# succinctlabs/tendermintx

Hardware: AMD Instinct MI355X
Metric: skip-circuit witness-gen ms at VALIDATOR_SET_SIZE_MAX=128 (lower is better)
Workload: dtype int64; 1 GPU; SkipCircuit VALIDATOR_SET_SIZE_MAX=128, batch of 256 proofs over 1 GPU(s) (BASELINE configs[3] batch per GPU, weak-scaled), 100 validators in 128 lanes, 4 distinct validator set(s) per batch, 90% sign; n_max=128, proofs_total=256, proofs_per_gpu=256, workload_name=survey8d, parallelism=proof-sharded x1, no data-path collective

## Files before the change

### include/tmx.h

```cpp
#ifndef TMX_H
#define TMX_H
#include <stddef.h>
#include <stdint.h>

#ifdef __cplusplus
extern "C" {
#endif

#define TMX_KIND_SKIP 0
#define TMX_KIND_STEP 1

#define TMX_N_MAX_LIMIT 512

#define TMX_VALIDATOR_MESSAGE_BYTES_LENGTH_MAX 124
#define TMX_VALIDATOR_BYTE_LENGTH_MAX 46
#define TMX_PROTOBUF_CHAIN_ID_SIZE_BYTES 52
#define TMX_HEADER_PROOF_DEPTH 4

#define TMX_FLAG_SIGNED 1u
#define TMX_FLAG_PRESENT 2u

typedef enum {
  TMX_OK = 0,
  TMX_ERR_BAD_ARG = -1,
// ... 443 lines not shown
#define TMX_TRACE_SHA256_HELPER 128u
#define TMX_TRACE_SHA256_QUOTIENT 256u
int32_t tmx_air_sha256_helper_device(tmx_ctx* ctx, uint32_t log_rows, uint32_t n_proofs, const uint64_t* d_table, uint64_t* d_helper,
                                     void* hip_stream);
int32_t tmx_air_sha256_quotient_device(tmx_ctx* ctx, uint32_t log_n, uint32_t log_blowup, uint32_t cap_height, uint32_t n_proofs,
                                       const uint64_t* d_cols, const uint64_t* d_helper_cols, const uint64_t* d_cap, const uint64_t* d_cap_helper,
                                       uint64_t* d_quot, void* hip_stream);
int32_t tmx_air_sha256_verify_device(tmx_ctx* ctx, const tmx_batch_params* p, uint32_t k_trace, const uint64_t* d_caps, const uint64_t* d_proof,
                                     uint32_t* d_ok, void* hip_stream);
int32_t tmx_trace_commit_set_air_sha256_device(tmx_ctx* ctx, uint32_t section, uint64_t* d_cap_h, uint64_t* d_cap_q, void* hip_stream);

int32_t tmx_selftest_fe_invert(tmx_ctx* ctx, uint32_t n, const uint32_t* in_words, uint32_t* out_words);

int32_t tmx_selftest_f16(tmx_ctx* ctx, uint32_t n, uint32_t doublings, const uint32_t* in_words, uint32_t* out_words);

#ifdef __cplusplus
}
#endif
#endif
```

### tendermintx_amd/_lib.py

```python
import ctypes as C
import ctypes.util
import importlib.util
import os
import sys

_HERE = os.path.dirname(os.path.abspath(__file__))
LIB_PATH = os.environ.get("TMX_LIB") or os.path.join(_HERE, "libtmx.so")

KIND_SKIP, KIND_STEP = 0, 1
FLAG_SIGNED, FLAG_PRESENT = 1, 2
N_KERNELS = 4
KERNEL_NAMES = ("k_eddsa", "k_proof", "k_verdict", "k_serialize")
ED_STRIDE = 448
SEC_HINT, SEC_DERIVED, SEC_ALL = 1, 2, 3
PROOF_PATH_NONE, PROOF_PATH_TINY, PROOF_PATH_ROLES, PROOF_PATH_R168, PROOF_PATH_K256, PROOF_PATH_WIDE = range(6)
TRACE_LADDERS, TRACE_SHA512, TRACE_SHA256, TRACE_MATCH, TRACE_TREE, TRACE_HEADER, TRACE_ALL = 1, 2, 4, 8, 16, 32, 63
TRACE_LADDERS_QUOTIENT = 64
AIR_SHA256_HELPER_COLS, AIR_SHA256_CONSTRAINTS = 300, 315
TRACE_SHA256_HELPER, TRACE_SHA256_QUOTIENT = 128, 256


class ValidatorRec(C.Structure):
    _fields_ = [("pubkey", C.c_uint8 * 32), ("signature", C.c_uint8 * 64), ("message", C.c_uint8 * 124),
                ("message_byte_length", C.c_uint16), ("validator_byte_length", C.c_uint8), ("flags", C.c_uint8),
# ... 270 lines not shown
        L.tmx_batch_verify_device.argtypes = [C.c_void_p, C.POINTER(BatchParams), C.c_void_p, C.c_void_p, C.c_void_p, C.c_void_p]
        L.tmx_trace_commit_set_device.argtypes = [C.c_void_p, C.c_int32, C.c_uint32, C.c_uint32, C.c_uint32, C.c_uint32, C.c_void_p, C.c_void_p,
                                                  C.c_void_p]
        L.tmx_trace_commit_set_shape.argtypes = [C.c_void_p, C.POINTER(BatchParams), C.POINTER(C.c_uint32)]
        L.tmx_trace_commit_set_prove_device.argtypes = [C.c_void_p, C.POINTER(BatchParams), C.c_void_p, C.c_void_p]
        L.tmx_trace_commit_set_bytes.argtypes = [C.c_int32] + [C.c_uint32] * 7
        L.tmx_trace_commit_set_bytes.restype = C.c_uint64
        L.tmx_trace_commit_set_streamed_device.argtypes = [C.c_void_p, C.c_int32, C.c_uint32, C.c_uint32, C.c_uint32, C.c_uint32, C.c_uint32,
                                                           C.c_uint32, C.c_void_p, C.c_void_p, C.c_void_p]
        L.tmx_air_ladder_quotient_device.argtypes = [C.c_void_p, C.c_uint32, C.c_uint32, C.c_uint32, C.c_uint32, C.c_void_p, C.c_void_p, C.c_void_p,
                                                     C.c_void_p]
        L.tmx_air_ladder_quotient_range_device.argtypes = [C.c_void_p] + [C.c_uint32] * 7 + [C.c_void_p] * 4
        L.tmx_air_last_gamma.argtypes = [C.c_void_p, C.POINTER(C.c_uint64)]
        L.tmx_air_verify_device.argtypes = [C.c_void_p, C.POINTER(BatchParams), C.c_uint32, C.c_void_p, C.c_void_p, C.c_void_p, C.c_void_p]
        L.tmx_trace_commit_set_air_device.argtypes = [C.c_void_p, C.c_void_p, C.c_void_p]
    except AttributeError:
        if not os.environ.get("TMX_LIB"):
            raise
    L.tmx_selftest_fe_invert.argtypes = [C.c_void_p, C.c_uint32, C.c_void_p, C.c_void_p]
    L.tmx_selftest_f16.argtypes = [C.c_void_p, C.c_uint32, C.c_uint32, C.c_void_p, C.c_void_p]
    L.tmx_eddsa_lanes_device.argtypes = [C.c_void_p, C.c_uint32, C.c_void_p, C.c_void_p, C.c_void_p]
    L.tmx_finish_batch_device.argtypes = [C.c_void_p, C.c_int32, C.c_uint32, C.c_void_p, C.c_void_p, C.c_void_p, C.c_void_p,
                                          C.c_void_p, C.c_void_p, C.c_void_p]
    L.tmx_trace_commit_shape.argtypes = [C.c_int32, C.c_uint32, C.c_uint32, C.POINTER(C.c_uint32), C.POINTER(C.c_uint32)]
    L.tmx_trace_commit_device.argtypes = [C.c_void_p, C.c_int32, C.c_uint32, C.c_uint32, C.c_uint32, C.c_uint32, C.c_void_p, C.c_void_p, C.c_void_p]
    L.tmx_trace_commit_last_ms.argtypes = [C.c_void_p, C.POINTER(C.c_float)]
    L.tmx_shard_range.restype = None
    L.tmx_shard_range.argtypes = [C.c_uint64, C.c_uint32, C.c_uint32, C.POINTER(C.c_uint64), C.POINTER(C.c_uint64)]
    L.tmx_comm_unique_id.argtypes = [C.c_char_p]
    L.tmx_comm_create.argtypes = [C.c_void_p, C.c_char_p, C.c_uint32, C.c_uint32]
# ... 83 lines not shown
```

### tendermintx_amd/context.py

```python
import ctypes as C

import numpy as np

from . import _lib
from ._lib import KIND_SKIP, KIND_STEP, Config, Report, check


def _indices(indices):
    if isinstance(indices, np.ndarray):
        return np.ascontiguousarray(indices.reshape(-1), dtype=np.uint64)
    return np.array([int(i) for i in indices], dtype=np.uint64)


class Context:

    def __init__(self, n_max, chain_id=b"celestia", skip_max=100800, device=0, max_batch=1):
        self._L = _lib.lib()
        self.n_max, self.chain_id, self.skip_max, self.max_batch = int(n_max), bytes(chain_id), int(skip_max), int(max_batch)
        cfg = Config()
        cfg.n_max = self.n_max
        cfg.chain_id_len = len(self.chain_id)
        for i, b in enumerate(self.chain_id[:52]):
            cfg.chain_id[i] = b
        cfg.skip_max = self.skip_max
# ... 151 lines not shown
        for i, v in enumerate(values):
            for k in range(8):
                inp[i, k] = (int(v) >> (32 * k)) & 0xFFFFFFFF
        out = np.zeros((n, 16), dtype=np.uint32)
        check(self._L.tmx_selftest_fe_invert(self._h, n, inp.ctypes.data, out.ctypes.data), self._h)
        conv = lambda w: sum(int(w[k]) << (32 * k) for k in range(8))
        return [(conv(out[i, :8]), conv(out[i, 8:])) for i in range(n)]

    def selftest_f16(self, words, doublings):
        inp = np.ascontiguousarray(words, dtype=np.uint32)
        n = inp.shape[0]
        out = np.zeros((n, 256), dtype=np.uint32)
        check(self._L.tmx_selftest_f16(self._h, n, doublings, inp.ctypes.data, out.ctypes.data), self._h)
        return out

    def ntt_set_domain(self, root_2_32, coset_shift):
        check(self._L.tmx_ntt_set_domain(self._h, C.c_uint64(root_2_32), C.c_uint64(coset_shift)), self._h)

    def ntt_device(self, log_n, n_cols, d_in, d_out, inverse=False, stream=None):
        check(self._L.tmx_ntt_goldilocks_device(self._h, log_n, n_cols, d_in, d_out, 1 if inverse else 0, self._stream(stream)), self._h)

    def lde_device(self, log_n, log_blowup, n_cols, d_in, d_out, stream=None):
        check(self._L.tmx_lde_goldilocks_device(self._h, log_n, log_blowup, n_cols, d_in, d_out, self._stream(stream)), self._h)

    def poseidon_set_constants(self, round_constants=None, mds_circ=None, mds_diag=None):
        arr = lambda v, n: (C.c_uint64 * n)(*[int(x) for x in v]) if v is not None else None
        check(self._L.tmx_poseidon_set_constants(self._h, arr(round_constants, 360), arr(mds_circ, 12), arr(mds_diag, 12)), self._h)

    def poseidon_permute(self, states):
        a = np.ascontiguousarray(states, dtype=np.uint64).reshape(-1, 12)
# ... 355 lines not shown
```

### tendermintx_amd/csrc/api.cpp

```cpp
#include <hip/hip_runtime_api.h>

#include <algorithm>
#include <chrono>
#include <cstdio>
#include <cstdlib>
#include <cstring>
#include <mutex>
#include <string>
#include <thread>
#include <vector>

#include "kernels.h"
#include "air.h"
#include "fri.h"
#include "ntt.h"
#include "poseidon.h"
#include "trace.h"
#include "tmx.h"
#include "value.h"

using namespace tmx;

static thread_local std::string g_tls_err;

// ... 2065 lines not shown
  HIPCK(c, hipSetDevice(c->cfg.device));
  void *d_in = nullptr, *d_out = nullptr;
  hipError_t e = hipMalloc(&d_in, (size_t)n * 512);
  if (e == hipSuccess) e = hipMalloc(&d_out, (size_t)n * 1024);
  if (e == hipSuccess) e = hipMemcpy(d_in, in_words, (size_t)n * 512, hipMemcpyHostToDevice);
  if (e == hipSuccess) e = hipMemsetAsync(d_out, 0, (size_t)n * 1024, c->side2);
  if (e == hipSuccess) e = (hipError_t)launch_selftest_f16(n, doublings, d_in, d_out, c->side2);
  if (e == hipSuccess) e = hipStreamSynchronize(c->side2);
  if (e == hipSuccess) e = hipMemcpy(out_words, d_out, (size_t)n * 1024, hipMemcpyDeviceToHost);
  if (d_in) (void)hipFree(d_in);
  if (d_out) (void)hipFree(d_out);
  if (e != hipSuccess) return fail(c, TMX_ERR_HIP, std::string("tmx_selftest_f16: ") + hipGetErrorString(e));
  return TMX_OK;
}

int32_t tmx_selftest_fe_invert(tmx_ctx* c, uint32_t n, const uint32_t* in_words, uint32_t* out_words) {
  if (!c || !in_words || !out_words) return TMX_ERR_BAD_ARG;
  if (n == 0) return TMX_OK;
  HIPCK(c, hipSetDevice(c->cfg.device));
  void *d_in = nullptr, *d_out = nullptr;
  hipError_t e = hipMalloc(&d_in, (size_t)n * 32);
  if (e == hipSuccess) e = hipMalloc(&d_out, (size_t)n * 64);
  if (e == hipSuccess) e = hipMemcpy(d_in, in_words, (size_t)n * 32, hipMemcpyHostToDevice);
  if (e == hipSuccess) e = (hipError_t)launch_selftest_invert(n, d_in, d_out, c->side2);
  if (e == hipSuccess) e = hipStreamSynchronize(c->side2);
  if (e == hipSuccess) e = hipMemcpy(out_words, d_out, (size_t)n * 64, hipMemcpyDeviceToHost);
  if (d_in) (void)hipFree(d_in);
  if (d_out) (void)hipFree(d_out);
  if (e != hipSuccess) return fail(c, TMX_ERR_HIP, std::string("tmx_selftest_fe_invert: ") + hipGetErrorString(e));
  return TMX_OK;
// ... 2305 lines not shown
```

### tendermintx_amd/csrc/fe25519.hpp

```cpp
#pragma once
#include <hip/hip_runtime.h>
#include <stdint.h>

namespace tmx {

struct fe {
  int32_t v[10];
};

#define TMX_DEV __device__ __forceinline__
#ifdef TMX_FE_NOINLINE
#define TMX_FE_FN __device__ __noinline__
#else
#define TMX_FE_FN __device__ __forceinline__
#endif

TMX_DEV fe fe_zero() {
  fe r;
#pragma unroll
  for (int i = 0; i < 10; i++) r.v[i] = 0;
  return r;
}
TMX_DEV fe fe_one() {
  fe r = fe_zero();
// ... 119 lines not shown
  r.v[1] += c;
  return r;
}

TMX_DEV fe fe_from_words(const uint32_t w[8]) {
  fe r;
  const int start[10] = {0, 26, 51, 77, 102, 128, 153, 179, 204, 230};
#pragma unroll
  for (int i = 0; i < 10; i++) {
    const int s = start[i], bits = (i & 1) ? 25 : 26;
    const int wi = s >> 5, sh = s & 31;
    uint64_t two = (uint64_t)w[wi] | ((wi + 1 < 8) ? ((uint64_t)w[wi + 1] << 32) : 0);
    uint32_t val = (uint32_t)(two >> sh) & ((1u << bits) - 1);
    if (i == 9) val &= (1u << 25) - 1;
    r.v[i] = (int32_t)val;
  }
  return r;
}

TMX_DEV void fe_to_words(const fe& a, uint32_t w[8]) {
  int32_t h[10];
#pragma unroll
  for (int i = 0; i < 10; i++) h[i] = a.v[i];
#pragma unroll
  for (int i = 0; i < 10; i++) {
    const int bits = (i & 1) ? 25 : 26;
    int32_t c = (h[i] + (1 << (bits - 1))) >> bits;
    h[i] -= c << bits;
    if (i < 9) h[i + 1] += c; else h[0] += 19 * c;
  }
// ... 98 lines not shown
```

### tendermintx_amd/csrc/kernels.h

```cpp
#pragma once
#include <stddef.h>
#include <stdint.h>

#include "layout.h"

namespace tmx {

struct KeyCache {
  uint32_t cap;
  uint32_t hash_mask;
  uint32_t new_cap;
  uint32_t persist;
  uint32_t* d_hash;
  uint32_t* d_pk;
  uint32_t* d_used;
  uint32_t* d_free;
  uint32_t* d_state;
  uint32_t* hint;
};
enum : uint32_t { KC_FREE_HEAD = 0, KC_N_FREE = 1, KC_EPOCH = 2, KC_RESIDENT = 3, KC_LAST_NEW = 4, KC_LAST_HIT_KEYS = 5, KC_LAST_HIT_LANES = 6,
                  KC_LAST_BUILT = 7, KC_LAST_USE_NEW = 8, KC_TOTALS = 16 , KC_STATE_WORDS = 32 };
enum : uint32_t { KC_TOT_HIT_LANES = 0, KC_TOT_MISS_LANES = 1, KC_TOT_BUILT = 2, KC_TOT_EVICTED = 3, KC_TOT_GC_RUNS = 4, KC_TOT_LAUNCHES = 5 };

size_t base_table_bytes();
int launch_init_base(void* d_table, void* stream);
int launch_selftest_invert(uint32_t n, const void* d_in, void* d_out, void* stream);
int launch_selftest_f16(uint32_t n, uint32_t doublings, const void* d_in, void* d_out, void* stream);
struct EdQuad {
  uint32_t n_lanes;
  const void* d_target;
  void* d_ed;
  uint32_t ed_stride;
  const void* d_qtable;
  void *d_pre, *d_mulout;
  void* d_hash;
  uint32_t hash_mask;
  void *d_cnt, *d_cnt_next, *d_owner_of, *d_slot_of_owner, *d_slot_of_uid, *d_owners, *d_keyrec, *d_anchors, *d_keytab;
  KeyCache kc;
  uint32_t mode;
  uint32_t use_new;
  uint32_t warm;
  RowOut row;
// ... 90 lines not shown
```

### tendermintx_amd/csrc/kernels.hip

```cpp
#include "kernels.h"

#include <hip/hip_runtime.h>
#include <hip/hip_ext.h>
#include <cstdlib>
#include <cstring>

#include <type_traits>

#include "ge25519.hpp"
#include "inv25519.hpp"
#include "fe16.hpp"
#include "winv25519.hpp"
#include "sc25519.hpp"
#include "sha2.hpp"

namespace tmx {

__device__ __forceinline__ uint32_t bswap32(uint32_t x) { return __builtin_bswap32(x); }
__device__ __forceinline__ uint32_t ld32(const uint8_t* p) { return *reinterpret_cast<const uint32_t*>(p); }
__device__ __forceinline__ uint64_t ld64(const uint8_t* p) { return *reinterpret_cast<const uint64_t*>(p); }
__device__ __forceinline__ void st32(uint8_t* p, uint32_t v) { *reinterpret_cast<uint32_t*>(p) = v; }
__device__ __forceinline__ void st64(uint8_t* p, uint64_t v) { *reinterpret_cast<uint64_t*>(p) = v; }

#ifdef TMX_WAVE_PROF
// ... 212 lines not shown
  const int32_t mR = (q == 0 || q == 2) ? (((q == 0) != neg) ? -1 : 0) : 0;
  const int32_t sL = mL & 1, sR = mR & 1;
  fe op1, op2;
#pragma unroll
  for (int i = 0; i < 10; i++) {
    op1.v[i] = dpp_quad<0x69>(r.v[i]) + (dpp_quad<0x3C>(r.v[i]) ^ mL) + sL;
    op2.v[i] = dpp_quad<0x66>(r.v[i]) + (dpp_quad<0x33>(r.v[i]) ^ mR) + sR;
  }
  return fe_mul(op1, op2);
}
__device__ __forceinline__ fe quad_to_cached(const fe& mine, int q) {
  fe bx = fe_qbcast<0>(mine), by = fe_qbcast<1>(mine);
  fe t2d = fe_mul(mine, K_2D);
  fe r = fe_select(fe_select(fe_select(t2d, fe_add(mine, mine), q == 2), fe_add(by, bx), q == 1), fe_sub(by, bx), q == 0);
  return fe_carry32(r);
}

constexpr uint32_t KEY_STRIDE = 256;
constexpr uint32_t KEY_OFF_A = 0, KEY_OFF_XY = 160, KEY_OFF_OK = 224;
constexpr uint32_t DEDUP_EMPTY = 0xffffffffu;
constexpr uint32_t KC_HIT = 0x80000000u;
constexpr uint32_t CNT_WORDS = 8, CNT_LIVE = 4;
__device__ __forceinline__ void effective_pk(const uint8_t* __restrict__ rec, uint32_t pk[8]) {
  const bool is_signed = rec[VR_OFF_FLAGS] & 1;
#pragma unroll
  for (int w = 0; w < 8; w++) pk[w] = is_signed ? ld32(rec + VR_OFF_PK + 4 * w) : K_DUMMY_PK[w];
}
__device__ __forceinline__ uint32_t pk_hash(const uint32_t pk[8]) {
  uint32_t hsh = 0x9e3779b9u;
#pragma unroll
// ... 385 lines not shown
  const fe P = load16(0);
  const fe cP = quad_to_cached(P, q);
  fe acc = fe_zero();
  acc.v[0] = (q == 1 || q == 2) ? 1 : 0;
  {
    bool first = true;
#pragma unroll
    for (int b = 0; b < KW - 4; b++) {
      if ((t >> b) & 1u) {
        const fe pb = load16(1 + b);
        acc = first ? pb : quad_add(acc, quad_to_cached(pb, q), q);
        first = false;
      }
    }
  }
  int32_t* tab = keytab + ((size_t)slot_of_uid[u] * C::NW + w) * C::HALF * 40;
  for (int j = 0; j < 8; j++) {
    acc = quad_add(acc, cP, q);
    const fe c = quad_to_cached(acc, q);
    int32_t* oj = tab + ((size_t)(8 * t + j) * 4 + q) * 10;
#pragma unroll
    for (int l = 0; l < 10; l++) oj[l] = c.v[l];
  }
  }
}
struct FusedCursor { uint32_t next, end, more; };
__device__ void fused_rows_step(const FusedRows& F, const SerializeProgram& S, FusedCursor& cur, uint32_t count, uint32_t chunk);

struct WalkArgs {
  uint32_t n_lanes, mode, use_new, cap;
  const uint32_t *cnt, *owner_of, *slot_of_owner, *pre;
  const int32_t* keytab;
  int32_t* mulout;
  uint32_t w0, w1;
  const uint32_t* live_list;
  uint32_t which;
};
// ... 18 lines not shown
  TMX_PROF(1);
  __builtin_amdgcn_s_setprio(2);
  int32_t* acc_mem = mulout + (size_t)lane * (MUL_STRIDE / 4) + 10 * q;
  fe mine = fe_zero();
  mine.v[0] = (q == 1 || q == 2) ? 1 : 0;
  if (walks && F == nullptr) {
    const uint32_t* po = pre + (size_t)lane * (PRE_STRIDE / 4);
    uint32_t h[8], e[C::NWORDS];
#pragma unroll
    for (int w = 0; w < 8; w++) h[w] = po[PRE_OFF_H / 4 + w];
    recode_signed_w<KW>(h, e);
    if (w0 != 0 && part == 0) {
#pragma unroll
      for (int i = 0; i < 10; i++) mine.v[i] = acc_mem[i];
    }
    const int32_t* tab = keytab + (size_t)slot * C::NW * C::HALF * 40;
    auto fetch = [&](int i, fe& c) {
      const int d = key_digit<KW>(e, i);
      const int m = d == 0 ? 0 : (d < 0 ? -d : d) - 1;
      const int32_t* ent = tab + (size_t)(i * C::HALF + m) * 40 + 10 * cached_component(q, d < 0);
#pragma unroll
      for (int l = 0; l < 10; l++) c.v[l] = ent[l];
    };
    const int span = (int)(w1 - w0);
    const int i0 = (int)w0 + (span * part + SPLIT - 1) / SPLIT, i1 = (int)w0 + (span * (part + 1) + SPLIT - 1) / SPLIT;
    fe cur;
    fetch(i0 < C::NW ? i0 : C::NW - 1, cur);
    for (int i = i0; i < i1; i++) {
      fe nxt;
      fetch(i < i1 - 1 ? i + 1 : i, nxt);
      const int d = key_digit<KW>(e, i);
      if (d != 0) mine = quad_add(mine, cur, q, d < 0);
      cur = nxt;
    }
  }
  if (F != nullptr) {
    const int span = (int)(w1 - w0);
    const int i0 = (int)w0 + (span * part + SPLIT - 1) / SPLIT, i1 = (int)w0 + (span * (part + 1) + SPLIT - 1) / SPLIT;
    const int steps = (span + SPLIT - 1) / SPLIT;
    const uint32_t* po = pre + (size_t)lane * (PRE_STRIDE / 4);
    uint32_t h[8], e[C::NWORDS];
#pragma unroll
    for (int w = 0; w < 8; w++) h[w] = walks ? po[PRE_OFF_H / 4 + w] : 0u;
    recode_signed_w<KW>(h, e);
    if (walks && w0 != 0 && part == 0) {
#pragma unroll
      for (int i = 0; i < 10; i++) mine.v[i] = acc_mem[i];
    }
    const int32_t* tab = keytab + (size_t)slot * C::NW * C::HALF * 40;
    auto fetch = [&](int i, fe& c) {
      const int d = key_digit<KW>(e, i);
      const int m = d == 0 ? 0 : (d < 0 ? -d : d) - 1;
      const int32_t* ent = tab + (size_t)(i * C::HALF + m) * 40 + 10 * cached_component(q, d < 0);
#pragma unroll
      for (int l = 0; l < 10; l++) c.v[l] = ent[l];
    };
    fe cur = fe_zero();
    if (walks) fetch(i0 < C::NW ? i0 : C::NW - 1, cur);
    FusedCursor fc = {0u, 0u, 1u};
    for (int k = 0; k < steps; k++) {
      const int i = i0 + k;
      fe nxt = cur;
      const bool act = walks && i < i1;
      if (act) fetch(i < i1 - 1 ? i + 1 : i, nxt);
      __builtin_amdgcn_sched_barrier(0);
      fused_rows_step(*F, *FS, fc, F->per_walk, F->per_walk * (uint32_t)steps);
      __builtin_amdgcn_sched_barrier(0);
      if (act) {
        const int d = key_digit<KW>(e, i);
        if (d != 0) mine = quad_add(mine, cur, q, d < 0);
      }
      cur = nxt;
    }
    fused_rows_step(*F, *FS, fc, fc.end - fc.next, 0u);
  }
#pragma unroll
  for (int step = 1; step < SPLIT; step *= 2) {
    fe c = quad_to_cached(mine, q), other;
#pragma unroll
    for (int l = 0; l < 10; l++) other.v[l] = __shfl_down(c.v[l], 4 * step, 64);
    mine = quad_add(mine, other, q);
  }
  if (live && walks && part == 0) {
#pragma unroll
    for (int i = 0; i < 10; i++) acc_mem[i] = mine.v[i];
// ... 83 lines not shown
  const uint32_t carry = recode_signed_w<W>(s, e);
  fe mine = fe_zero();
  mine.v[0] = (q == 1 || q == 2) ? 1 : 0;
  FusedCursor fc = {0u, 0u, F != nullptr ? 1u : 0u};
  for (int wi = 0; wi < C::NWORDS; wi++) {
    uint32_t word = e[0];
#pragma unroll
    for (int w = 1; w < C::NWORDS; w++) word = (wi == w) ? e[w] : word;
    for (int sl = 0; sl < C::PER; sl++) {
      const int i = wi * C::PER + sl;
      if (i >= C::NW) break;
      const int d = __builtin_amdgcn_sbfe((int)word, W * sl, W);
      if (F == nullptr) {
        if (d != 0) {
          const int m = (d < 0 ? -d : d) - 1;
          const int32_t* ent = qtable + ((size_t)(i * C::HALF + m) * 4 + cached_component(q, d < 0)) * 10;
          fe c;
#pragma unroll
          for (int l = 0; l < 10; l++) c.v[l] = ent[l];
          mine = quad_add(mine, c, q, d < 0);
        }
      } else {
        const int m = d == 0 ? 0 : (d < 0 ? -d : d) - 1;
        const int32_t* ent = qtable + ((size_t)(i * C::HALF + m) * 4 + cached_component(q, d < 0)) * 10;
        fe c;
#pragma unroll
        for (int l = 0; l < 10; l++) c.v[l] = ent[l];
        __builtin_amdgcn_sched_barrier(0);
        fused_rows_step(*F, *FS, fc, F->per_base, F->per_base * (uint32_t)C::NW);
        __builtin_amdgcn_sched_barrier(0);
        if (d != 0) mine = quad_add(mine, c, q, d < 0);
      }
    }
  }
  if (F != nullptr) fused_rows_step(*F, *FS, fc, fc.end - fc.next, 0u);
  if (carry) {
    const int32_t* ent = qtable + ((size_t)(C::ENTRIES - 1) * 4 + q) * 10;
    fe c;
#pragma unroll
    for (int l = 0; l < 10; l++) c.v[l] = ent[l];
    mine = quad_add(mine, c, q);
  }
  if (live) {
    int32_t* o = mulout + (size_t)lane * (MUL_STRIDE / 4) + 40 + 10 * q;
#pragma unroll
    for (int i = 0; i < 10; i++) o[i] = mine.v[i];
  }
}

template <int W>
__global__ __launch_bounds__(64) void k_ed_phase1(uint32_t n_lanes, const uint8_t* __restrict__ in_target, uint32_t* __restrict__ pre,
                                                  uint8_t* __restrict__ ed, uint32_t ed_stride, const int32_t* __restrict__ qtable,
                                                  int32_t* __restrict__ mulout, const uint32_t* __restrict__ live_list, const uint32_t* __restrict__ cnt) {
  const uint32_t nbl = (n_lanes + 63) / 64;
  const uint32_t b = blockIdx.x;
  __builtin_amdgcn_s_setprio(2);
// ... 33 lines not shown
template <int W>
__global__ __launch_bounds__(64) void k_ed_base_rows(uint32_t n_lanes, const uint8_t* __restrict__ in_target, const int32_t* __restrict__ qtable,
                                                     int32_t* __restrict__ mulout, const uint32_t* __restrict__ live_list, const uint32_t* __restrict__ cnt,
                                                     FusedRows F, SerializeProgram FS) {
  TMX_PROF(3);
  uint32_t lane;
  const bool live = compact_lane(live_list, cnt, n_lanes, blockIdx.x * 16 + (threadIdx.x >> 2), lane);
  if (__ballot(live) == 0) return;
  ed_role_base<W>(lane, live, threadIdx.x & 3, in_target + (size_t)lane * VR_STRIDE, qtable, mulout, &F, &FS);
}

__global__ __launch_bounds__(64) void k_init_base_quad(const ge_affc* __restrict__ table, int32_t* __restrict__ qtable, uint32_t n_entries) {
  uint32_t t = blockIdx.x * blockDim.x + threadIdx.x;
  if (t >= n_entries) return;
  ge_affc e = table[t];
  int32_t* o = qtable + (size_t)t * 40;
#pragma unroll
  for (int i = 0; i < 10; i++) { o[i] = e.ymx.v[i]; o[10 + i] = e.ypx.v[i]; o[20 + i] = (i == 0) ? 2 : 0; o[30 + i] = e.xy2d.v[i]; }
}

__global__ __launch_bounds__(64) void k_ed_mul(uint32_t n_lanes, uint32_t mode, uint32_t use_new, uint32_t cap, const uint32_t* __restrict__ cnt,
                                               const uint32_t* __restrict__ owner_of, const uint32_t* __restrict__ slot_of_owner,
                                               const uint32_t* __restrict__ keyrec, const uint32_t* __restrict__ pre,
                                               int32_t* __restrict__ mulout, const uint8_t* __restrict__ skip_unsigned) {
  __shared__ int32_t s_tab[8][10][64];
  const int tid = threadIdx.x, q = tid & 3;
  uint32_t lane = blockIdx.x * 16 + (tid >> 2);
  const bool live = lane < n_lanes;
  if (!live) lane = n_lanes - 1;
  bool walks;
  const uint32_t slot = lane_slot(owner_of, slot_of_owner, lane, cap, kc_use_new(cnt, mode, n_lanes, use_new), walks);
  if (skip_unsigned && !(skip_unsigned[(size_t)lane * VR_STRIDE + VR_OFF_FLAGS] & 1)) walks = true;
  if (__ballot(live && !walks) == 0) return;
// ... 1391 lines not shown
    int32_t l10[10];
#pragma unroll
    for (int l = 0; l < 16; l++) l16[l] = in[128 * i + 16 * tid + l];
    f16::to_limbs10(l16, l10);
#pragma unroll
    for (int l = 0; l < 10; l++) out[256 * i + 128 + 10 * tid + l] = (uint32_t)l10[l];
  }
  out[256 * i + 192 + tid] = f16::from_limbs10(reinterpret_cast<const int32_t*>(in + 128 * i + 64 + 10 * c.row), c);
}
int launch_selftest_f16(uint32_t n, uint32_t d, const void* d_in, void* d_out, void* stream) {
  if (n == 0) return 0;
  hipLaunchKernelGGL(k_selftest_f16, dim3(n), dim3(64), 0, S_(stream), n, d, reinterpret_cast<const uint32_t*>(d_in),
                     reinterpret_cast<uint32_t*>(d_out));
  return (int)hipGetLastError();
}
int launch_selftest_invert(uint32_t n, const void* d_in, void* d_out, void* stream) {
  if (n == 0) return 0;
  hipLaunchKernelGGL(k_selftest_invert, dim3((n + 63) / 64), dim3(64), 0, S_(stream), n, reinterpret_cast<const uint32_t*>(d_in),
                     reinterpret_cast<uint32_t*>(d_out));
  return (int)hipGetLastError();
}
int launch_init_base(void* d_table, void* stream) {
  hipLaunchKernelGGL(k_init_base, dim3((BASE_ENTRIES + 63) / 64), dim3(64), 0, S_(stream), reinterpret_cast<ge_affc*>(d_table), (uint32_t)BASE_W, BASE_ENTRIES);
  return (int)hipGetLastError();
}
size_t base_table_bytes() { return sizeof(ge_affc) * BASE_ENTRIES; }

size_t quad_table_bytes() { return (size_t)BASE_ENTRIES * 40 * 4; }
size_t pre_bytes_per_lane() { return PRE_STRIDE; }
size_t mulout_bytes_per_lane() { return MUL_STRIDE; }
int launch_init_base_quad(const void* d_table, void* d_qtable, void* stream) {
  hipLaunchKernelGGL(k_init_base_quad, dim3((BASE_ENTRIES + 63) / 64), dim3(64), 0, S_(stream), reinterpret_cast<const ge_affc*>(d_table),
                     reinterpret_cast<int32_t*>(d_qtable), BASE_ENTRIES);
  return (int)hipGetLastError();
}
int launch_valid_skip(uint32_t n_cand, uint32_t n_max, const void* d_start, uint32_t n_start, const void* d_targets, const void* d_nt, const void* d_sigs,
                      const void* d_ns, void* d_valid, void* d_shared, void* d_total, void* stream) {
  if (n_cand == 0) return 0;
  hipLaunchKernelGGL(k_valid_skip, dim3(n_cand), dim3(256), 0, S_(stream), n_max, reinterpret_cast<const uint8_t*>(d_start), n_start,
                     reinterpret_cast<const uint8_t*>(d_targets), reinterpret_cast<const uint32_t*>(d_nt), reinterpret_cast<const uint8_t*>(d_sigs),
                     reinterpret_cast<const uint32_t*>(d_ns), reinterpret_cast<uint8_t*>(d_valid), reinterpret_cast<uint64_t*>(d_shared),
                     reinterpret_cast<uint64_t*>(d_total));
  return (int)hipGetLastError();
}
size_t key_bytes_per_key() { return KEY_STRIDE; }
#ifndef TMX_KEY_W
#define TMX_KEY_W 8
#endif
constexpr int KEY_W = TMX_KEY_W;
size_t anchor_bytes_per_key() { return (size_t)KeyWin<KEY_W>::NW * anchor_words<KEY_W>() * 4; }
size_t keytab_bytes_per_key() { return (size_t)KeyWin<KEY_W>::NW * KeyWin<KEY_W>::HALF * 40 * 4; }
int launch_kc_reset(const KeyCache& kc, void* stream) {
  hipLaunchKernelGGL(k_kc_reset, dim3(256), dim3(256), 0, S_(stream), kc);
  return (int)hipGetLastError();
}

int launch_ed_dedup(const EdQuad& Q, void* stream, void* done) {
  if (Q.n_lanes == 0) return 0;
  hipExtLaunchKernelGGL(k_ed_dedup, dim3((Q.n_lanes + 255) / 256), dim3(256), 0, S_(stream), nullptr, E_(done), 0, Q.n_lanes, reinterpret_cast<const uint8_t*>(Q.d_target),
                     reinterpret_cast<uint32_t*>(Q.d_hash), Q.hash_mask, reinterpret_cast<uint32_t*>(Q.d_cnt), reinterpret_cast<uint32_t*>(Q.d_cnt_next),
                     reinterpret_cast<uint32_t*>(Q.d_owner_of), reinterpret_cast<uint32_t*>(Q.d_owners), Q.kc, Q.mode,
                     Q.compact ? reinterpret_cast<uint32_t*>(Q.d_live) : nullptr, reinterpret_cast<const uint32_t*>(Q.d_dummy_ed), reinterpret_cast<uint8_t*>(Q.d_ed),
                     Q.ed_stride, Q.row);
  return (int)hipGetLastError();
}
#ifndef TMX_WARM_BUILD_KEYS
// ... 367 lines not shown
```

### tendermintx_amd/csrc/tiny.hpp

```cpp
#pragma once

constexpr uint32_t TINY_THREADS = 128;
#ifdef TMX_TINY_PROF
#define TINY_DBG(bit) (g_tiny_dbg & (bit))
__device__ uint32_t g_tiny_dbg;
#else
#define TINY_DBG(bit) false
#endif
enum : uint32_t { TN_WORDS = 8, TN_PER_PROOF = 16 };

struct TinyEd {
  uint32_t n_lanes;
  const uint8_t* in_target;
  uint8_t* ed;
  uint32_t ed_stride;
  const int32_t* qtable;
  const int32_t* keytab;
  const uint32_t* keyrec;
  KeyCache kc;
  RowOut row;
  uint32_t* tiny;
  uint8_t* shadow;
};
struct TinyProof {
// ... 30 lines not shown
  }
  return mine;
}
template <int W>
__device__ __forceinline__ fe tiny_base(const uint8_t* __restrict__ rec, const int32_t* __restrict__ qtable, int q, int part) {
  using C = BaseWin<W>;
  const bool is_signed = rec[VR_OFF_FLAGS] & 1;
  uint32_t s[8], e[C::NWORDS];
#pragma unroll
  for (int w = 0; w < 8; w++) s[w] = is_signed ? ld32(rec + VR_OFF_SIG + 32 + 4 * w) : K_DUMMY_SIG[8 + w];
  const uint32_t carry = recode_signed_w<W>(s, e);
  fe mine = fe_zero();
  mine.v[0] = (q == 1 || q == 2) ? 1 : 0;
  constexpr int PERP = (C::NW + 15) / 16;
  const int i0 = (C::NW * part + 15) / 16, i1 = (C::NW * (part + 1) + 15) / 16;
  fe ent[PERP];
  int dg[PERP];
#pragma unroll
  for (int k = 0; k < PERP; k++) {
    const int i = i0 + k;
    const int d = i < i1 ? key_digit_v<W>(e, i) : 0;
    dg[k] = d;
    const int m = d == 0 ? 0 : (d < 0 ? -d : d) - 1;
    const int32_t* src = qtable + ((size_t)((i < C::NW ? i : C::NW - 1) * C::HALF + m) * 4 + cached_component(q, d < 0)) * 10;
#pragma unroll
    for (int l = 0; l < 10; l++) ent[k].v[l] = src[l];
  }
#pragma unroll
  for (int k = 0; k < PERP; k++)
    if (dg[k] != 0) mine = quad_add(mine, ent[k], q, dg[k] < 0);
  if (carry && part == 0) {
    const int32_t* src = qtable + ((size_t)(C::ENTRIES - 1) * 4 + q) * 10;
    fe c;
#pragma unroll
    for (int l = 0; l < 10; l++) c.v[l] = src[l];
    mine = quad_add(mine, c, q);
  }
  return quad_merge16(mine, q);
}
template <int KW>
__device__ __forceinline__ fe tiny_walk(const uint32_t* h_lds, const int32_t* __restrict__ tab, int q, int part) {
  using C = KeyWin<KW>;
  uint32_t h[8], e[C::NWORDS];
#pragma unroll
  for (int w = 0; w < 8; w++) h[w] = h_lds[w];
  recode_signed_w<KW>(h, e);
  fe mine = fe_zero();
  mine.v[0] = (q == 1 || q == 2) ? 1 : 0;
  constexpr int PERP = (C::NW + 15) / 16;
  const int i0 = (C::NW * part + 15) / 16, i1 = (C::NW * (part + 1) + 15) / 16;
  fe ent[PERP];
  int dg[PERP];
#pragma unroll
  for (int k = 0; k < PERP; k++) {
    const int i = i0 + k;
    const int d = i < i1 ? key_digit_v<KW>(e, i) : 0;
    dg[k] = d;
    const int m = d == 0 ? 0 : (d < 0 ? -d : d) - 1;
    const int32_t* src = tab + (size_t)((i < C::NW ? i : C::NW - 1) * C::HALF + m) * 40 + 10 * cached_component(q, d < 0);
#pragma unroll
    for (int l = 0; l < 10; l++) ent[k].v[l] = src[l];
  }
#pragma unroll
  for (int k = 0; k < PERP; k++)
    if (dg[k] != 0) mine = quad_add(mine, ent[k], q, dg[k] < 0);
  return quad_merge16(mine, q);
}

struct TinyLaneLds {
  int32_t pt[2][40];
  uint32_t h[8];
  uint32_t key[64];
  uint32_t slot;
  uint32_t sh[6][64];
  uint64_t w[2][80];
  uint32_t h16[6][8];
};

__device__ __forceinline__ void tiny_hram(const uint8_t* __restrict__ rec, uint8_t* __restrict__ o, TinyLaneLds& L, uint32_t blk) {
  const bool is_signed = rec[VR_OFF_FLAGS] & 1;
// ... 208 lines not shown
      T = fe_select(T, fe_neg(T), flip);
      fe_to_words(X, xw);
      key_store(L.key, X, fe_carry32(fe_from_words(pk)), T, xw, (ok_direct || ok_flipped) && !(x_zero && sign));
    }
    __syncthreads();
  }
  if (tid >= 64) {
    const int t1 = (int)tid - 64, q = t1 & 3, part = t1 >> 2;
    const fe sB = tiny_base<BW>(rec, A.qtable, q, part);
    if (part == 0) {
#pragma unroll
      for (int i = 0; i < 10; i++) L.pt[1][10 * q + i] = sB.v[i];
    }
  } else if (hit) {
    const int q = (int)tid & 3, part = (int)tid >> 2;
    const fe hA = tiny_walk<KW>(L.h, A.keytab + (size_t)slot * KeyWin<KW>::NW * KeyWin<KW>::HALF * 40, q, part);
    if (part == 0) {
#pragma unroll
      for (int i = 0; i < 10; i++) L.pt[0][10 * q + i] = hA.v[i];
    }
  } else {
    uint32_t h[8], e[8];
#pragma unroll
    for (int w = 0; w < 8; w++) h[w] = L.h[w];
    recode_signed16(h, e);
    const u32x8 ev = vec8_of(e);
    const uint32_t Ak = f16::from_limbs10(reinterpret_cast<const int32_t*>(L.key + KEY_OFF_A / 4 + 10 * c.row), c);
    uint32_t tab[8], Q;
    tab[0] = f16::to_cached(Ak, c);
    f16::dbl(f16::with_xy(Ak, c), Q, c);
    tab[1] = f16::to_cached(Q, c);
// ... 557 lines not shown
```

Measured before the change: 1.424 us.

## Pack precomputed point tables into 256-bit words with vector loads

Changes the base and per-key cached point tables from ten 32-bit limbs per component to packed 8-word (256-bit) representations, 32 words per entry instead of 40. Table reads become two 16-byte vector loads, unpacked to limbs with alignbit. The constant Z=2 component is synthesized instead of loaded. This cuts table memory and bandwidth for the scalar-multiplication walks, at the cost of extra unpack ALU work and pack work when tables are built. A selftest kernel is added for the new pack/unpack path.

```diff
diff --git a/include/tmx.h b/include/tmx.h
--- a/include/tmx.h
+++ b/include/tmx.h
@@ -481,6 +481,8 @@
 
 int32_t tmx_selftest_f16(tmx_ctx* ctx, uint32_t n, uint32_t doublings, const uint32_t* in_words, uint32_t* out_words);
 
+int32_t tmx_selftest_tab_pack(tmx_ctx* ctx, uint32_t n, const uint32_t* in_words, uint32_t* out_words);
+
 #ifdef __cplusplus
 }
 #endif
diff --git a/tendermintx_amd/_lib.py b/tendermintx_amd/_lib.py
--- a/tendermintx_amd/_lib.py
+++ b/tendermintx_amd/_lib.py
@@ -308,6 +308,7 @@
         L.tmx_air_last_gamma.argtypes = [C.c_void_p, C.POINTER(C.c_uint64)]
         L.tmx_air_verify_device.argtypes = [C.c_void_p, C.POINTER(BatchParams), C.c_uint32, C.c_void_p, C.c_void_p, C.c_void_p, C.c_void_p]
         L.tmx_trace_commit_set_air_device.argtypes = [C.c_void_p, C.c_void_p, C.c_void_p]
+        L.tmx_selftest_tab_pack.argtypes = [C.c_void_p, C.c_uint32, C.c_void_p, C.c_void_p]
     except AttributeError:
         if not os.environ.get("TMX_LIB"):
             raise
diff --git a/tendermintx_amd/context.py b/tendermintx_amd/context.py
--- a/tendermintx_amd/context.py
+++ b/tendermintx_amd/context.py
@@ -189,6 +189,18 @@
         check(self._L.tmx_selftest_f16(self._h, n, doublings, inp.ctypes.data, out.ctypes.data), self._h)
         return out
 
+    def selftest_tab_pack(self, values, others):
+        n = len(values)
+        inp = np.zeros((n, 16), dtype=np.uint32)
+        for i, (a, b) in enumerate(zip(values, others)):
+            for k in range(8):
+                inp[i, k] = (int(a) >> (32 * k)) & 0xFFFFFFFF
+                inp[i, 8 + k] = (int(b) >> (32 * k)) & 0xFFFFFFFF
+        out = np.zeros((n, 32), dtype=np.uint32)
+        check(self._L.tmx_selftest_tab_pack(self._h, n, inp.ctypes.data, out.ctypes.data), self._h)
+        conv = lambda w: sum(int(w[k]) << (32 * k) for k in range(8))
+        return [(conv(out[i, :8]), [int(x) for x in out[i, 8:18]], conv(out[i, 18:26])) for i in range(n)]
+
     def ntt_set_domain(self, root_2_32, coset_shift):
         check(self._L.tmx_ntt_set_domain(self._h, C.c_uint64(root_2_32), C.c_uint64(coset_shift)), self._h)
 
diff --git a/tendermintx_amd/csrc/api.cpp b/tendermintx_amd/csrc/api.cpp
--- a/tendermintx_amd/csrc/api.cpp
+++ b/tendermintx_amd/csrc/api.cpp
@@ -2103,6 +2103,24 @@
   return TMX_OK;
 }
 
+int32_t tmx_selftest_tab_pack(tmx_ctx* c, uint32_t n, const uint32_t* in_words, uint32_t* out_words) {
+  if (!c || !in_words || !out_words) return TMX_ERR_BAD_ARG;
+  if (n == 0) return TMX_OK;
+  HIPCK(c, hipSetDevice(c->cfg.device));
+  void *d_in = nullptr, *d_out = nullptr;
+  hipError_t e = hipMalloc(&d_in, (size_t)n * 64);
+  if (e == hipSuccess) e = hipMalloc(&d_out, (size_t)n * 128);
+  if (e == hipSuccess) e = hipMemcpy(d_in, in_words, (size_t)n * 64, hipMemcpyHostToDevice);
+  if (e == hipSuccess) e = hipMemsetAsync(d_out, 0, (size_t)n * 128, c->side2);
+  if (e == hipSuccess) e = (hipError_t)launch_selftest_tab_pack(n, d_in, d_out, c->side2);
+  if (e == hipSuccess) e = hipStreamSynchronize(c->side2);
+  if (e == hipSuccess) e = hipMemcpy(out_words, d_out, (size_t)n * 128, hipMemcpyDeviceToHost);
+  if (d_in) (void)hipFree(d_in);
+  if (d_out) (void)hipFree(d_out);
+  if (e != hipSuccess) return fail(c, TMX_ERR_HIP, std::string("tmx_selftest_tab_pack: ") + hipGetErrorString(e));
+  return TMX_OK;
+}
+
 int32_t tmx_selftest_fe_invert(tmx_ctx* c, uint32_t n, const uint32_t* in_words, uint32_t* out_words) {
   if (!c || !in_words || !out_words) return TMX_ERR_BAD_ARG;
   if (n == 0) return TMX_OK;
diff --git a/tendermintx_amd/csrc/fe25519.hpp b/tendermintx_amd/csrc/fe25519.hpp
--- a/tendermintx_amd/csrc/fe25519.hpp
+++ b/tendermintx_amd/csrc/fe25519.hpp
@@ -157,6 +157,19 @@
     uint32_t val = (uint32_t)(two >> sh) & ((1u << bits) - 1);
     if (i == 9) val &= (1u << 25) - 1;
     r.v[i] = (int32_t)val;
+  }
+  return r;
+}
+
+TMX_DEV fe fe_unpack(const uint32_t w[8]) {
+  fe r;
+  const int start[10] = {0, 26, 51, 77, 102, 128, 153, 179, 204, 230};
+#pragma unroll
+  for (int i = 0; i < 10; i++) {
+    const int s = start[i], bits = (i & 1) ? 25 : 26;
+    const int wi = s >> 5, sh = s & 31;
+    const uint32_t raw = (sh + bits <= 32) ? (w[wi] >> sh) : __builtin_amdgcn_alignbit(w[wi + 1 < 8 ? wi + 1 : 7], w[wi], sh);
+    r.v[i] = (int32_t)(raw & ((1u << bits) - 1));
   }
   return r;
 }
diff --git a/tendermintx_amd/csrc/kernels.h b/tendermintx_amd/csrc/kernels.h
--- a/tendermintx_amd/csrc/kernels.h
+++ b/tendermintx_amd/csrc/kernels.h
@@ -26,6 +26,7 @@
 int launch_init_base(void* d_table, void* stream);
 int launch_selftest_invert(uint32_t n, const void* d_in, void* d_out, void* stream);
 int launch_selftest_f16(uint32_t n, uint32_t doublings, const void* d_in, void* d_out, void* stream);
+int launch_selftest_tab_pack(uint32_t n, const void* d_in, void* d_out, void* stream);
 struct EdQuad {
   uint32_t n_lanes;
   const void* d_target;
diff --git a/tendermintx_amd/csrc/kernels.hip b/tendermintx_amd/csrc/kernels.hip
--- a/tendermintx_amd/csrc/kernels.hip
+++ b/tendermintx_amd/csrc/kernels.hip
@@ -250,6 +250,27 @@
   fe t2d = fe_mul(mine, K_2D);
   fe r = fe_select(fe_select(fe_select(t2d, fe_add(mine, mine), q == 2), fe_add(by, bx), q == 1), fe_sub(by, bx), q == 0);
   return fe_carry32(r);
+}
+
+constexpr int TAB_ENTRY_WORDS = 32;
+struct fe_packed { uint32_t w[8]; };
+__device__ __forceinline__ void tab_load(const int32_t* __restrict__ ent, int comp, fe_packed& c) {
+  const uint4* p = reinterpret_cast<const uint4*>(ent) + 2 * comp;
+  const uint4 lo = p[0], hi = p[1];
+  c.w[0] = lo.x; c.w[1] = lo.y; c.w[2] = lo.z; c.w[3] = lo.w;
+  c.w[4] = hi.x; c.w[5] = hi.y; c.w[6] = hi.z; c.w[7] = hi.w;
+}
+__device__ __forceinline__ void tab_store(int32_t* __restrict__ ent, int comp, const fe& v) {
+  uint32_t w[8];
+  fe_to_words(v, w);
+  uint4* p = reinterpret_cast<uint4*>(ent) + 2 * comp;
+  p[0] = make_uint4(w[0], w[1], w[2], w[3]);
+  p[1] = make_uint4(w[4], w[5], w[6], w[7]);
+}
+__device__ __forceinline__ void base_load(const int32_t* __restrict__ qtable, size_t entry, int q, bool neg, fe_packed& c) {
+#pragma unroll
+  for (int k = 0; k < 8; k++) c.w[k] = k == 0 ? 2u : 0u;
+  if (q != 2) tab_load(qtable + entry * TAB_ENTRY_WORDS, q == 3 ? 2 : cached_component(q, neg), c);
 }
 
 constexpr uint32_t KEY_STRIDE = 256;
@@ -665,13 +686,10 @@
       }
     }
   }
-  int32_t* tab = keytab + ((size_t)slot_of_uid[u] * C::NW + w) * C::HALF * 40;
+  int32_t* tab = keytab + ((size_t)slot_of_uid[u] * C::NW + w) * C::HALF * TAB_ENTRY_WORDS;
   for (int j = 0; j < 8; j++) {
     acc = quad_add(acc, cP, q);
-    const fe c = quad_to_cached(acc, q);
-    int32_t* oj = tab + ((size_t)(8 * t + j) * 4 + q) * 10;
-#pragma unroll
-    for (int l = 0; l < 10; l++) oj[l] = c.v[l];
+    tab_store(tab + (size_t)(8 * t + j) * TAB_ENTRY_WORDS, q, quad_to_cached(acc, q));
   }
   }
 }
@@ -720,23 +738,21 @@
 #pragma unroll
       for (int i = 0; i < 10; i++) mine.v[i] = acc_mem[i];
     }
-    const int32_t* tab = keytab + (size_t)slot * C::NW * C::HALF * 40;
-    auto fetch = [&](int i, fe& c) {
+    const int32_t* tab = keytab + (size_t)slot * C::NW * C::HALF * TAB_ENTRY_WORDS;
+    auto fetch = [&](int i, fe_packed& c) {
       const int d = key_digit<KW>(e, i);
       const int m = d == 0 ? 0 : (d < 0 ? -d : d) - 1;
-      const int32_t* ent = tab + (size_t)(i * C::HALF + m) * 40 + 10 * cached_component(q, d < 0);
-#pragma unroll
-      for (int l = 0; l < 10; l++) c.v[l] = ent[l];
+      tab_load(tab + (size_t)(i * C::HALF + m) * TAB_ENTRY_WORDS, cached_component(q, d < 0), c);
     };
     const int span = (int)(w1 - w0);
     const int i0 = (int)w0 + (span * part + SPLIT - 1) / SPLIT, i1 = (int)w0 + (span * (part + 1) + SPLIT - 1) / SPLIT;
-    fe cur;
+    fe_packed cur;
     fetch(i0 < C::NW ? i0 : C::NW - 1, cur);
     for (int i = i0; i < i1; i++) {
-      fe nxt;
+      fe_packed nxt;
       fetch(i < i1 - 1 ? i + 1 : i, nxt);
       const int d = key_digit<KW>(e, i);
-      if (d != 0) mine = quad_add(mine, cur, q, d < 0);
+      if (d != 0) mine = quad_add(mine, fe_unpack(cur.w), q, d < 0);
       cur = nxt;
     }
   }
@@ -753,20 +769,18 @@
 #pragma unroll
       for (int i = 0; i < 10; i++) mine.v[i] = acc_mem[i];
     }
-    const int32_t* tab = keytab + (size_t)slot * C::NW * C::HALF * 40;
-    auto fetch = [&](int i, fe& c) {
+    const int32_t* tab = keytab + (size_t)slot * C::NW * C::HALF * TAB_ENTRY_WORDS;
+    auto fetch = [&](int i, fe_packed& c) {
       const int d = key_digit<KW>(e, i);
       const int m = d == 0 ? 0 : (d < 0 ? -d : d) - 1;
-      const int32_t* ent = tab + (size_t)(i * C::HALF + m) * 40 + 10 * cached_component(q, d < 0);
-#pragma unroll
-      for (int l = 0; l < 10; l++) c.v[l] = ent[l];
+      tab_load(tab + (size_t)(i * C::HALF + m) * TAB_ENTRY_WORDS, cached_component(q, d < 0), c);
     };
-    fe cur = fe_zero();
+    fe_packed cur = {};
     if (walks) fetch(i0 < C::NW ? i0 : C::NW - 1, cur);
     FusedCursor fc = {0u, 0u, 1u};
     for (int k = 0; k < steps; k++) {
       const int i = i0 + k;
-      fe nxt = cur;
+      fe_packed nxt = cur;
       const bool act = walks && i < i1;
       if (act) fetch(i < i1 - 1 ? i + 1 : i, nxt);
       __builtin_amdgcn_sched_barrier(0);
@@ -774,7 +788,7 @@
       __builtin_amdgcn_sched_barrier(0);
       if (act) {
         const int d = key_digit<KW>(e, i);
-        if (d != 0) mine = quad_add(mine, cur, q, d < 0);
+        if (d != 0) mine = quad_add(mine, fe_unpack(cur.w), q, d < 0);
       }
       cur = nxt;
     }
@@ -888,32 +902,26 @@
       if (F == nullptr) {
         if (d != 0) {
           const int m = (d < 0 ? -d : d) - 1;
-          const int32_t* ent = qtable + ((size_t)(i * C::HALF + m) * 4 + cached_component(q, d < 0)) * 10;
-          fe c;
-#pragma unroll
-          for (int l = 0; l < 10; l++) c.v[l] = ent[l];
-          mine = quad_add(mine, c, q, d < 0);
+          fe_packed c;
+          base_load(qtable, (size_t)(i * C::HALF + m), q, d < 0, c);
+          mine = quad_add(mine, fe_unpack(c.w), q, d < 0);
         }
       } else {
         const int m = d == 0 ? 0 : (d < 0 ? -d : d) - 1;
-        const int32_t* ent = qtable + ((size_t)(i * C::HALF + m) * 4 + cached_component(q, d < 0)) * 10;
-        fe c;
-#pragma unroll
-        for (int l = 0; l < 10; l++) c.v[l] = ent[l];
+        fe_packed c;
+        base_load(qtable, (size_t)(i * C::HALF + m), q, d < 0, c);
         __builtin_amdgcn_sched_barrier(0);
         fused_rows_step(*F, *FS, fc, F->per_base, F->per_base * (uint32_t)C::NW);
         __builtin_amdgcn_sched_barrier(0);
-        if (d != 0) mine = quad_add(mine, c, q, d < 0);
+        if (d != 0) mine = quad_add(mine, fe_unpack(c.w), q, d < 0);
       }
     }
   }
   if (F != nullptr) fused_rows_step(*F, *FS, fc, fc.end - fc.next, 0u);
   if (carry) {
-    const int32_t* ent = qtable + ((size_t)(C::ENTRIES - 1) * 4 + q) * 10;
-    fe c;
-#pragma unroll
-    for (int l = 0; l < 10; l++) c.v[l] = ent[l];
-    mine = quad_add(mine, c, q);
+    fe_packed c;
+    base_load(qtable, (size_t)(C::ENTRIES - 1), q, false, c);
+    mine = quad_add(mine, fe_unpack(c.w), q);
   }
   if (live) {
     int32_t* o = mulout + (size_t)lane * (MUL_STRIDE / 4) + 40 + 10 * q;
@@ -977,9 +985,12 @@
   uint32_t t = blockIdx.x * blockDim.x + threadIdx.x;
   if (t >= n_entries) return;
   ge_affc e = table[t];
-  int32_t* o = qtable + (size_t)t * 40;
-#pragma unroll
-  for (int i = 0; i < 10; i++) { o[i] = e.ymx.v[i]; o[10 + i] = e.ypx.v[i]; o[20 + i] = (i == 0) ? 2 : 0; o[30 + i] = e.xy2d.v[i]; }
+  int32_t* o = qtable + (size_t)t * TAB_ENTRY_WORDS;
+  tab_store(o, 0, e.ymx);
+  tab_store(o, 1, e.ypx);
+  tab_store(o, 2, e.xy2d);
+  reinterpret_cast<uint4*>(o)[6] = make_uint4(0u, 0u, 0u, 0u);
+  reinterpret_cast<uint4*>(o)[7] = make_uint4(0u, 0u, 0u, 0u);
 }
 
 __global__ __launch_bounds__(64) void k_ed_mul(uint32_t n_lanes, uint32_t mode, uint32_t use_new, uint32_t cap, const uint32_t* __restrict__ cnt,
@@ -2401,6 +2412,31 @@
                      reinterpret_cast<uint32_t*>(d_out));
   return (int)hipGetLastError();
 }
+__global__ __launch_bounds__(64) void k_selftest_tab_pack(uint32_t n, const uint32_t* __restrict__ in, uint32_t* __restrict__ out) {
+  const uint32_t i = blockIdx.x * blockDim.x + threadIdx.x;
+  if (i >= n) return;
+  uint32_t wa[8], wb[8];
+#pragma unroll
+  for (int k = 0; k < 8; k++) { wa[k] = in[16 * i + k]; wb[k] = in[16 * i + 8 + k]; }
+  int32_t* ent = reinterpret_cast<int32_t*>(out + (size_t)TAB_ENTRY_WORDS * i);
+  tab_store(ent, 0, fe_from_words(wa));
+  __threadfence();
+  fe_packed c;
+  tab_load(ent, 0, c);
+  const fe u = fe_unpack(c.w);
+  uint32_t wp[8];
+  fe_to_words(fe_mul(u, fe_from_words(wb)), wp);
+#pragma unroll
+  for (int l = 0; l < 10; l++) out[32 * i + 8 + l] = (uint32_t)u.v[l];
+#pragma unroll
+  for (int k = 0; k < 8; k++) out[32 * i + 18 + k] = wp[k];
+}
+int launch_selftest_tab_pack(uint32_t n, const void* d_in, void* d_out, void* stream) {
+  if (n == 0) return 0;
+  hipLaunchKernelGGL(k_selftest_tab_pack, dim3((n + 63) / 64), dim3(64), 0, S_(stream), n, reinterpret_cast<const uint32_t*>(d_in),
+                     reinterpret_cast<uint32_t*>(d_out));
+  return (int)hipGetLastError();
+}
 int launch_selftest_invert(uint32_t n, const void* d_in, void* d_out, void* stream) {
   if (n == 0) return 0;
   hipLaunchKernelGGL(k_selftest_invert, dim3((n + 63) / 64), dim3(64), 0, S_(stream), n, reinterpret_cast<const uint32_t*>(d_in),
@@ -2413,7 +2449,7 @@
 }
 size_t base_table_bytes() { return sizeof(ge_affc) * BASE_ENTRIES; }
 
-size_t quad_table_bytes() { return (size_t)BASE_ENTRIES * 40 * 4; }
+size_t quad_table_bytes() { return (size_t)BASE_ENTRIES * TAB_ENTRY_WORDS * 4; }
 size_t pre_bytes_per_lane() { return PRE_STRIDE; }
 size_t mulout_bytes_per_lane() { return MUL_STRIDE; }
 int launch_init_base_quad(const void* d_table, void* d_qtable, void* stream) {
@@ -2436,7 +2472,7 @@
 #endif
 constexpr int KEY_W = TMX_KEY_W;
 size_t anchor_bytes_per_key() { return (size_t)KeyWin<KEY_W>::NW * anchor_words<KEY_W>() * 4; }
-size_t keytab_bytes_per_key() { return (size_t)KeyWin<KEY_W>::NW * KeyWin<KEY_W>::HALF * 40 * 4; }
+size_t keytab_bytes_per_key() { return (size_t)KeyWin<KEY_W>::NW * KeyWin<KEY_W>::HALF * TAB_ENTRY_WORDS * 4; }
 int launch_kc_reset(const KeyCache& kc, void* stream) {
   hipLaunchKernelGGL(k_kc_reset, dim3(256), dim3(256), 0, S_(stream), kc);
   return (int)hipGetLastError();
diff --git a/tendermintx_amd/csrc/tiny.hpp b/tendermintx_amd/csrc/tiny.hpp
--- a/tendermintx_amd/csrc/tiny.hpp
+++ b/tendermintx_amd/csrc/tiny.hpp
@@ -68,7 +68,7 @@
   mine.v[0] = (q == 1 || q == 2) ? 1 : 0;
   constexpr int PERP = (C::NW + 15) / 16;
   const int i0 = (C::NW * part + 15) / 16, i1 = (C::NW * (part + 1) + 15) / 16;
-  fe ent[PERP];
+  fe_packed ent[PERP];
   int dg[PERP];
 #pragma unroll
   for (int k = 0; k < PERP; k++) {
@@ -76,19 +76,15 @@
     const int d = i < i1 ? key_digit_v<W>(e, i) : 0;
     dg[k] = d;
     const int m = d == 0 ? 0 : (d < 0 ? -d : d) - 1;
-    const int32_t* src = qtable + ((size_t)((i < C::NW ? i : C::NW - 1) * C::HALF + m) * 4 + cached_component(q, d < 0)) * 10;
-#pragma unroll
-    for (int l = 0; l < 10; l++) ent[k].v[l] = src[l];
+    base_load(qtable, (size_t)((i < C::NW ? i : C::NW - 1) * C::HALF + m), q, d < 0, ent[k]);
   }
 #pragma unroll
   for (int k = 0; k < PERP; k++)
-    if (dg[k] != 0) mine = quad_add(mine, ent[k], q, dg[k] < 0);
+    if (dg[k] != 0) mine = quad_add(mine, fe_unpack(ent[k].w), q, dg[k] < 0);
   if (carry && part == 0) {
-    const int32_t* src = qtable + ((size_t)(C::ENTRIES - 1) * 4 + q) * 10;
-    fe c;
-#pragma unroll
-    for (int l = 0; l < 10; l++) c.v[l] = src[l];
-    mine = quad_add(mine, c, q);
+    fe_packed c;
+    base_load(qtable, (size_t)(C::ENTRIES - 1), q, false, c);
+    mine = quad_add(mine, fe_unpack(c.w), q);
   }
   return quad_merge16(mine, q);
 }
@@ -103,7 +99,7 @@
   mine.v[0] = (q == 1 || q == 2) ? 1 : 0;
   constexpr int PERP = (C::NW + 15) / 16;
   const int i0 = (C::NW * part + 15) / 16, i1 = (C::NW * (part + 1) + 15) / 16;
-  fe ent[PERP];
+  fe_packed ent[PERP];
   int dg[PERP];
 #pragma unroll
   for (int k = 0; k < PERP; k++) {
@@ -111,13 +107,11 @@
     const int d = i < i1 ? key_digit_v<KW>(e, i) : 0;
     dg[k] = d;
     const int m = d == 0 ? 0 : (d < 0 ? -d : d) - 1;
-    const int32_t* src = tab + (size_t)((i < C::NW ? i : C::NW - 1) * C::HALF + m) * 40 + 10 * cached_component(q, d < 0);
-#pragma unroll
-    for (int l = 0; l < 10; l++) ent[k].v[l] = src[l];
+    tab_load(tab + (size_t)((i < C::NW ? i : C::NW - 1) * C::HALF + m) * TAB_ENTRY_WORDS, cached_component(q, d < 0), ent[k]);
   }
 #pragma unroll
   for (int k = 0; k < PERP; k++)
-    if (dg[k] != 0) mine = quad_add(mine, ent[k], q, dg[k] < 0);
+    if (dg[k] != 0) mine = quad_add(mine, fe_unpack(ent[k].w), q, dg[k] < 0);
   return quad_merge16(mine, q);
 }
 
@@ -356,7 +350,7 @@
     }
   } else if (hit) {
     const int q = (int)tid & 3, part = (int)tid >> 2;
-    const fe hA = tiny_walk<KW>(L.h, A.keytab + (size_t)slot * KeyWin<KW>::NW * KeyWin<KW>::HALF * 40, q, part);
+    const fe hA = tiny_walk<KW>(L.h, A.keytab + (size_t)slot * KeyWin<KW>::NW * KeyWin<KW>::HALF * TAB_ENTRY_WORDS, q, part);
     if (part == 0) {
 #pragma unroll
       for (int i = 0; i < 10; i++) L.pt[0][10 * q + i] = hA.v[i];
```

Result: faster. 1.382 us (median of 6 runs) (-3.0%).
